# ztaylor797/APMBackend

Hardware: AMD Instinct MI355X
Metric: log-lines/sec z-scored (whole node) (higher is better)
Workload: dtype fp64

## Files before the change

apmbackend_amd/csrc/kernels/common.h:

```cpp
#pragma once
#include <cstring>
#include <cstdio>
#include <cstdlib>
#include <hip/hip_runtime.h>
#include <stdint.h>
#include <math.h>

#include "../apm_types.h"

#define APM_WAVE 64

#define HIP_OK(x)                                                                      \
  do {                                                                                 \
    hipError_t _e = (x);                                                               \
    if (_e != hipSuccess) {                                                            \
      fprintf(stderr, "HIP error %s at %s:%d: %s\n", hipGetErrorName(_e), __FILE__,    \
              __LINE__, hipGetErrorString(_e));                                        \
      abort();                                                                         \
    }                                                                                  \
  } while (0)

namespace apm {

__host__ __device__ inline double apm_nan() { return __builtin_nan(""); }
// ... 9 lines not shown
}

__host__ __device__ inline int64_t floordiv64(int64_t a, int64_t b) {
  int64_t q = a / b;
  if ((a % b != 0) && ((a < 0) != (b < 0))) --q;
  return q;
}

__host__ __device__ inline int64_t make_date_ms(int64_t y, int64_t mon0, int64_t d, int64_t h,
                                                int64_t mi, int64_t s, int64_t ms) {
  const int64_t ym = y + floordiv64(mon0, 12);
  const int64_t mn = mon0 - floordiv64(mon0, 12) * 12;
  const int64_t day = days_from_civil(ym, mn + 1, 1) + d - 1;
  return day * 86400000LL + ((h * 60 + mi) * 60 + s) * 1000 + ms;
}

struct TzTable {
  int n;
  int64_t local_start[64];
  int64_t offset_ms[64];
};

__host__ __device__ inline int64_t local_to_utc(const TzTable& tz, int64_t local_ms) {
  int lo = 0, hi = tz.n - 1;
  while (lo < hi) {
    int mid = (lo + hi + 1) >> 1;
    if (tz.local_start[mid] <= local_ms) lo = mid; else hi = mid - 1;
  }
  return local_ms - tz.offset_ms[lo];
}

__host__ __device__ inline double js_round_fixed(double x, int f) {
  if (x != x) return x;
  const double scale = f == 0 ? 1.0 : (f == 1 ? 10.0 : (f == 2 ? 100.0 : 1000.0));
  const bool neg = x < 0;
  const double ax = neg ? -x : x;
  if (ax >= 1e21) return x;
  const double p = ax * scale;
  const double e = fma(ax, scale, -p);
  const double q = floor(p);
  const double d = (p - q) - 0.5;
  double n = q;
  if (d > 0 || (d == 0 && e >= 0)) n = q + 1;
  double r = n / scale;
  return neg ? -r : r;
}

constexpr int HIST_BINS = 120;
__host__ __device__ inline int hist_bin(int32_t v) {
  if (v < 4) return v <= 0 ? 0 : v;
  const int e = 31 - __builtin_clz((uint32_t)v);
  return 4 * (e - 1) + (int)(((uint32_t)v >> (e - 2)) & 3u);
}
__host__ __device__ inline uint32_t hist_lower(int b) {
  return b < 4 ? (uint32_t)b : (uint32_t)(4 + (b & 3)) << (b / 4 - 1);
}

__host__ __device__ inline uint64_t hash_mix(uint64_t a, uint64_t b) {
  const __uint128_t r = (__uint128_t)a * b;
  return (uint64_t)r ^ (uint64_t)(r >> 64);
}

constexpr uint64_t kHashSeed = 0x243f6a8885a308d3ULL;
constexpr uint64_t kHashSeedEjb = 0x13198a2e03707344ULL;

__host__ __device__ inline uint64_t hash_bytes(const void* data, size_t n, uint64_t seed = kHashSeed) {
  const uint8_t* p = static_cast<const uint8_t*>(data);
  uint64_t h = seed ^ hash_mix(n ^ 0xa0761d6478bd642fULL, 0xe7037ed1a0b428dbULL);
  while (n >= 8) {
    uint64_t w;
    memcpy(&w, p, 8);
    h = hash_mix(h ^ w, 0x8ebc6af09c88c6e3ULL);
    p += 8;
    n -= 8;
  }
  if (n) {
    uint64_t w = 0;
    memcpy(&w, p, n);
    h = hash_mix(h ^ w ^ ((uint64_t)n << 59), 0x589965cc75374cc3ULL);
  }
  return hash_mix(h, 0x1d8e4e27c47d124fULL);
}

__host__ __device__ inline uint64_t fnv1a64(const uint8_t* p, int n, uint64_t h = 1469598103934665603ULL) {
  for (int i = 0; i < n; ++i) { h ^= p[i]; h *= 1099511628211ULL; }
  return h;
}

}
```

apmbackend_amd/csrc/kernels/devjoin.hip:

```cpp
#include "kernel_api.h"

#include <rocprim/rocprim.hpp>

#include <chrono>
#include <climits>
#include <cstdlib>
#include <cstddef>
#include <cstring>
#include <vector>

#include "devjoin_api.h"
#include "devjoin_dev.h"
#include "devscan.h"
#include "prim.h"
#include "textout.h"

namespace apm {
using namespace dj;

namespace {

constexpr int TB = 256;

__device__ __forceinline__ uint32_t grid_n(uint32_t n) { return (n + TB - 1) / TB; }

constexpr uint32_t AUD_NIL = 0xffffffffu;

__device__ __forceinline__ bool ws_ascii(uint8_t c) { return c == ' ' || (c >= 9 && c <= 13); }

__device__ __forceinline__ void trim_ascii(const uint8_t* p, int& a, int& b) {
  while (a < b && ws_ascii(p[a])) ++a;
  while (b > a && ws_ascii(p[b - 1])) --b;
}

__device__ bool parse_int_nobr(const uint8_t* p, int a, int b, double& out) {
  uint64_t x = 0;
  int nd = 0, k = 0;
  for (int i = a; i < b; ++i) {
    const uint8_t ch = p[i];
    if (ch == '[' || ch == ']') continue;
    if (k == 0 && (ch == '+' || ch == '-')) return false;
    if (k == 1 && nd == 1 && x == 0 && (ch == 'x' || ch == 'X')) return false;
    ++k;
    if (ch < '0' || ch > '9') break;
    if (nd >= 19) return false;
    x = x * 10 + (ch - '0');
    ++nd;
  }
  out = nd == 0 ? apm_nan() : (double)x;
  return true;
}

__device__ int aud_date(const uint8_t* p, int a, int b, double& out) {
  if (a >= b) return 1;
  int tpos = -1;
  for (int i = a; i < b; ++i) if (p[i] == 'T') { tpos = i; break; }
  bool iso = false;
  if (tpos >= 0) for (int i = tpos + 1; i < b; ++i) if (p[i] == '-') { iso = true; break; }
  if (!iso) return -1;
  trim_ascii(p, a, b);
  const int n = b - a;
  const uint8_t* t = p + a;
  auto dig = [&](int i, int k, int64_t& v) {
    if (i + k > n) return false;
    v = 0;
    for (int j = 0; j < k; ++j) {
      const uint8_t c = t[i + j];
      if (c < '0' || c > '9') return false;
      v = v * 10 + (c - '0');
    }
    return true;
  };
  out = apm_nan();
  int64_t y, mo, d, h, mi, sec = 0, ms = 0;
  if (!dig(0, 4, y) || n < 16 || t[4] != '-' || !dig(5, 2, mo) || t[7] != '-' || !dig(8, 2, d) || t[10] != 'T' ||
      !dig(11, 2, h) || t[13] != ':' || !dig(14, 2, mi))
    return 0;
  int i = 16;
  if (i < n && t[i] == ':') {
    if (!dig(i + 1, 2, sec)) return 0;
    i += 3;
    if (i < n && t[i] == '.') {
      ++i;
      int j = i, nd = 0;
      int64_t frac = 0;
      while (j < n && t[j] >= '0' && t[j] <= '9') { if (nd < 3) { frac = frac * 10 + (t[j] - '0'); ++nd; } ++j; }
      if (j == i) return 0;
      while (nd < 3) { frac *= 10; ++nd; }
      ms = frac;
      i = j;
    }
  }
  if (mo < 1 || mo > 12 || d < 1 || d > 31 || h > 24 || mi > 59 || sec > 59) return 0;
  const int64_t local = make_date_ms(y, mo - 1, d, h, mi, sec, ms);
  if (i == n) return -1;
  if (t[i] == 'Z' && i + 1 == n) { out = (double)local; return 0; }
  if (t[i] == '+' || t[i] == '-') {
    const int sg = t[i] == '-' ? -1 : 1;
    int64_t oh, om;
    if (!dig(i + 1, 2, oh)) return 0;
    int k = i + 3;
    if (k < n && t[k] == ':') ++k;
    if (!dig(k, 2, om) || k + 2 != n) return 0;
    out = (double)(local - sg * (oh * 60 + om) * 60000);
  }
  return 0;
}

__device__ bool icontains_provider(const uint8_t* p, int a, int b) {
  const char* pat = "provider[";
  for (int i = a; i + 9 <= b; ++i) {
    int k = 0;
    for (; k < 9; ++k) {
      uint8_t c = p[i + k];
      if (c >= 'A' && c <= 'Z') c = (uint8_t)(c + 32);
      if (c != (uint8_t)pat[k]) break;
    }
    if (k == 9) return true;
  }
  return false;
}

struct LineScan {
  bool nonascii;
  int c1, c2;
  int t0s, t0e, t3s, t3e, t5s, t5e;
  int eq1, eq2;
  int lt, gt;
};

__device__ void line_scan(const uint8_t* __restrict__ p, int len, LineScan& L) {
  bool na = false;
  int c1 = -1, c2 = len;
  int t0s = -1, t0e = -1, t3s = -1, t3e = -1, t5s = -1, t5e = -1;
  int eq1 = -1, eq2 = -1, lt = len, gt = -1;
  int tok = 0, tstart = 0;
  bool in_ws = false, lt_found = false;
  uint8_t prev = 0;
  const uintptr_t a0 = (uintptr_t)p & ~(uintptr_t)15;
  const int lead = (int)((uintptr_t)p - a0);
  for (int base = -lead; base < len; base += 16) {
    const uint4 v = *reinterpret_cast<const uint4*>(p + base);
    const uint32_t w4[4] = {v.x, v.y, v.z, v.w};
#pragma unroll
    for (int j = 0; j < 16; ++j) {
      const int i = base + j;
      if (i < 0 || i >= len) continue;
      const uint8_t c = (uint8_t)(w4[j >> 2] >> (8 * (j & 3)));
      na |= c >= 0x80;
      if (c == ':') {
        if (c1 < 0) c1 = i;
        else if (c2 == len) c2 = i;
      }
      if (!lt_found) {
        if (prev == '<' && c == '/') { lt = i - 1; lt_found = true; }
        else if (c == '>') gt = i;
      }
      if (ws_ascii(c)) {
        if (!in_ws) {
          if (tok == 0) { t0s = tstart; t0e = i; }
          else if (tok == 3) { t3s = tstart; t3e = i; }
          else if (tok == 5) { t5s = tstart; t5e = i; }
          ++tok;
          in_ws = true;
        }
        tstart = i + 1;
      } else {
        in_ws = false;
        if (tok == 5 && c == '=') {
          if (eq1 < 0) eq1 = i + 1;
          else if (eq2 < 0) eq2 = i;
        }
      }
      prev = c;
    }
  }
  if (tok == 0) { t0s = tstart; t0e = len; }
  else if (tok == 3) { t3s = tstart; t3e = len; }
  else if (tok == 5) { t5s = tstart; t5e = len; }
  if (eq1 >= 0 && eq2 < 0) eq2 = t5e;
  L.nonascii = na; L.c1 = c1; L.c2 = c2;
  L.t0s = t0s; L.t0e = t0e; L.t3s = t3s; L.t3e = t3e; L.t5s = t5s; L.t5e = t5e;
  L.eq1 = eq1; L.eq2 = eq2; L.lt = lt; L.gt = gt;
}

__device__ bool baf_account_scan(const uint8_t* p, int a, int b, int& n, bool& digits, double& v) {
  int st = a;
  for (int i = a; i + 1 < b; ++i) if (p[i] == ']' && p[i + 1] == '[') st = i + 2;
  int c = st;
  for (int i = st; i < b; ++i) if (p[i] == ':') c = i + 1;
  n = 0;
  digits = true;
  uint64_t x = 0;
  int nd = 0;
  bool in_digits = true;
  for (int i = c; i < b; ++i) {
    const uint8_t ch = p[i];
    if (ch == '[' || ch == ']') continue;
    const bool d = ch >= '0' && ch <= '9';
    if (n == 0 && (ch == '+' || ch == '-')) return false;
    if (n == 1 && nd == 1 && x == 0 && (ch == 'x' || ch == 'X')) return false;
    digits &= d;
    if (in_digits) {
      if (d) {
        if (nd >= 19) return false;
        x = x * 10 + (ch - '0');
        ++nd;
      } else {
        in_digits = false;
      }
    }
    ++n;
  }
  v = nd == 0 ? apm_nan() : (double)x;
  if (n == 0) digits = false;
  return true;
}

__device__ bool aud_fields(const Event& e, const uint8_t* __restrict__ p, uint64_t fkey, AudF& f) {
  const int len = (int)e.len;
  f.h_item = 0; f.el = apm_nan(); f.h_sw = 0; f.ts = apm_nan();
  f.ref = 0; f.len = 0; f.flags = 0; f.pad = 0; f.pad2[0] = f.pad2[1] = 0;
  LineScan L;
  line_scan(p, len, L);
  if (L.nonascii) return false;
  const uint32_t m = e.mask;
  if (m & PM_AUTR_MAP) {
    int s0 = L.t0s, e0 = L.t0e;
    if (s0 < 0) { s0 = e0 = 0; }
    if (s0 < e0 && p[s0] == '[') ++s0;
    if (e0 > s0 && p[e0 - 1] == ']') --e0;
    for (int i = s0; i < e0; ++i) if (p[i] == '[' || p[i] == ']') return false;
    f.ref = e.off + (uint32_t)s0;
    f.len = (uint16_t)(e0 - s0);
    f.h_sw = hash_bytes(p + s0, (size_t)(e0 - s0));
    const uint64_t ah = L.eq1 < 0 ? hash_bytes("undefined", 9) : hash_bytes(p + L.eq1, (size_t)(L.eq2 - L.eq1));
    f.h_item = aud_key(ah, fkey);
    if ((m & PM_BAF) && L.t3s >= 0 && L.t3e > L.t3s) {
      int n;
      bool digits;
      double v;
      if (!baf_account_scan(p, L.t3s, L.t3e, n, digits, v)) return false;
      if (n > 0) {
        f.el = v;
        f.flags |= AF_ACCT;
        if (digits) f.flags |= AF_ACCT_VALID;
      }
    }
    return true;
  }
  if (m & PM_AUTR_HDR) {
    if (L.c1 < 0) return false;
    int a = L.c1 + 1, b = L.c2;
    trim_ascii(p, a, b);
    f.h_item = aud_key(hash_bytes(p + a, (size_t)(b - a)), fkey);
    return true;
  }
  {
    int a = 0, b = L.c1 >= 0 ? L.c1 : len;
    trim_ascii(p, a, b);
    f.h_item = hash_bytes(p + a, (size_t)(b - a));
    if (L.c1 >= 0) {
      int t = L.c1 + 1;
      while (t < L.c2 && !ws_ascii(p[t])) ++t;
      if (!parse_int_nobr(p, L.c1 + 1, t, f.el)) return false;
    }
  }
  if (m & (PM_SW_NAME | PM_SW_STARTTS | PM_SW_STOPTS)) {
    const int t = L.lt, s = L.gt >= 0 ? L.gt + 1 : 0;
    if (m & PM_SW_NAME) {
      f.ref = e.off + (uint32_t)s;
      f.len = (uint16_t)(t - s);
      f.h_sw = hash_bytes(p + s, (size_t)(t - s));
      if (!icontains_provider(p, s, t)) f.flags |= AF_TO_DB;
    } else {
      const int r = aud_date(p, s, t, f.ts);
      if (r < 0) return false;
      if (r == 1) f.flags |= AF_TS_EMPTY;
    }
  }
  return true;
}

enum : uint8_t { PRE_BAF = 1, PRE_BAF_VALID = 2, PRE_SOAP_VALID = 4 };
__device__ __forceinline__ uint32_t zero_bytes(uint32_t x) {
  return ~((((x & 0x7f7f7f7fu) + 0x7f7f7f7fu) | x) | 0x7f7f7f7fu);
}
__device__ void angle_field2_dev(const uint8_t* __restrict__ p, int len, int& fs, int& fe) {
  auto ws = [](uint8_t c) { return c == ' ' || (c >= 9 && c <= 13); };
  int a = 0, b = len;
  while (a < b && ws(p[a])) ++a;
  while (b > a && ws(p[b - 1])) --b;
  fs = fe = -1;
  int seen = 0, start = -1;
  const int lead = (int)((uintptr_t)(p + a) & 15u);
  const uint4* q = reinterpret_cast<const uint4*>(p + a - lead);
  for (int g = a - lead; g < b; g += 16, ++q) {
    const uint4 v = *q;
    const uint32_t w[4] = {v.x, v.y, v.z, v.w};
#pragma unroll
    for (int k = 0; k < 4; ++k) {
      uint32_t m = zero_bytes(w[k] ^ 0x3c3c3c3cu) | zero_bytes(w[k] ^ 0x3e3e3e3eu);
      while (m) {
        const int i = g + 4 * k + (__builtin_ctz(m) >> 3);
        m &= m - 1;
        if (i < a || i >= b) continue;
        if (seen == 2) { fs = start; fe = i; return; }
        if (++seen == 2) start = i + 1;
      }
    }
  }
  if (seen == 2) { fs = start; fe = b; }
}

__device__ int pre_fields(const Event& e, const uint8_t* __restrict__ p, AudF& f) {
  if (e.mask & PM_HOST) return -1;
  f.h_item = 0; f.el = apm_nan(); f.h_sw = 0; f.ts = apm_nan(); f.ref = 0; f.len = 0; f.flags = 0; f.pad = 0;
  if (e.kind >= LK_EJB_ENTRY && e.kind <= LK_CT_EXIT) {
    if (!(e.mask & PM_KEYS) || e.ntok < 3) return -1;
    if (e.kind == LK_CT_EXIT && (e.mask & PM_BAF)) {
      int n = 9;
      bool digits = false;
      double v = apm_nan();
      if (e.ntok >= 4 && !baf_account_scan(p, e.t3s, e.t3e, n, digits, v)) return -1;
      f.el = v;
      f.flags = (uint8_t)((n > 0 ? PRE_BAF : 0) | (digits ? PRE_BAF_VALID : 0));
      return 1;
    }
    return 0;
  }
  if (e.kind == LK_SOAP) {
    const uint32_t m = e.mask;
    if (m & PM_SOAP_IN) {
      int s = -1, t = -1;
      if (e.ntok >= 2) {
        const int a0 = e.t1s, b0 = e.t1e;
        for (int k = a0; k < b0; ++k) if (p[k] == '=') { s = k + 1; break; }
        if (s >= 0) { t = b0; for (int k = s; k < b0; ++k) if (p[k] == '=') { t = k; break; } }
      }
      f.h_item = s >= 0 ? hash_bytes(p + s, (size_t)(t - s)) : hash_bytes("undefined", 9, kHashSeedEjb);
      return 1;
    }
    if (m & PM_SOAP_OUT) return 0;
    if (m & (PM_SOAP_ACCT | PM_SOAP_VALUE)) {
      if (!(m & PM_SOAP_ACCT) && (m & PM_SOAP_KEY)) return 0;
      int fs, fe;
      angle_field2_dev(p, (int)e.len, fs, fe);
      if (fs >= 0) {
        while (fs < fe && (p[fs] == ' ' || (p[fs] >= 9 && p[fs] <= 13))) ++fs;
        while (fe > fs && (p[fe - 1] == ' ' || (p[fe - 1] >= 9 && p[fe - 1] <= 13))) --fe;
        if (all_digits(p + fs, fe - fs)) {
          double v;
          if (!simple_parse_int(p + fs, fe - fs, v)) return -1;
          f.el = v;
          f.flags = PRE_SOAP_VALID;
        }
      }
      return 1;
    }
  }
  return 0;
}

enum : uint8_t { SEL_HOST = 1, SEL_MH = 2, SEL_WALK = 4 };

constexpr int SEL_MH_SHIFT = 22, SEL_WALK_SHIFT = 43;
__device__ __forceinline__ SelCount sel_unpack(uint64_t v) {
  return SelCount{(uint32_t)(v & ((1ull << SEL_MH_SHIFT) - 1)),
                  (uint32_t)((v >> SEL_MH_SHIFT) & ((1ull << (SEL_WALK_SHIFT - SEL_MH_SHIFT)) - 1)),
                  (uint32_t)(v >> SEL_WALK_SHIFT), 0u};
}

constexpr int HF_SLOT = 256;
constexpr int HF_PITCH = HF_SLOT + 16;

__device__ __forceinline__ bool hf_needs_bytes(const Event& e) {
  if (e.kind == LK_APP) return !(e.mask & PM_HOST);
  if (e.mask & PM_HOST) return false;
  if (e.kind == LK_CT_EXIT) return (e.mask & PM_KEYS) && e.ntok >= 3 && (e.mask & PM_BAF);
  if (e.kind == LK_SOAP) return (e.mask & (PM_SOAP_IN | PM_SOAP_ACCT | PM_SOAP_VALUE)) != 0;
  return false;
}

__device__ __forceinline__ uint8_t hf_fields(const Event& e, const uint8_t* __restrict__ p, uint64_t fkey, AudF* aud,
                                             uint32_t i) {
  uint8_t fl = 0;
  if (e.kind == LK_APP) {
    bool host = (e.mask & PM_HOST) != 0;
    if (!host) {
      AudF f;
      host = !aud_fields(e, p, fkey, f);
      if (!host) aud[i] = f;
    }
    if (host) fl |= SEL_HOST;
  } else {
    AudF f;
    const int r = pre_fields(e, p, f);
    if (r < 0) fl |= SEL_HOST;
    else if (r > 0) aud[i] = f;
  }
  return fl;
}

__device__ __forceinline__ uint32_t wave_append(bool want, uint32_t* counter) {
  const uint64_t m = __ballot(want);
  if (!m) return ~0u;
  const uint32_t lane = threadIdx.x & (APM_WAVE - 1);
  const uint32_t leader = (uint32_t)__ffsll((unsigned long long)m) - 1u;
  uint32_t base = 0;
  if (lane == leader) base = atomicAdd(counter, (uint32_t)__popcll(m));
  base = (uint32_t)__shfl((int)base, (int)leader, APM_WAVE);
  return want ? base + (uint32_t)__popcll(m & ((1ull << lane) - 1ull)) : ~0u;
}

__device__ __forceinline__ uint64_t sel_pack(uint8_t fl) {
  return (uint64_t)(fl & SEL_HOST) | ((fl & SEL_MH) ? 1ull << SEL_MH_SHIFT : 0ull) |
         ((fl & SEL_WALK) ? 1ull << SEL_WALK_SHIFT : 0ull);
}

__device__ __forceinline__ uint8_t app_bits(const Event& e) {
  if (e.kind != LK_APP) return 0;
  return (e.mask & PM_AUTR_MAP) ? SEL_MH : (uint8_t)(SEL_WALK | ((e.mask & PM_AUTR_HDR) ? SEL_MH : 0));
}

__device__ __forceinline__ uint8_t hf_event(const Event& e, uint32_t i, const uint8_t* __restrict__ bytes,
                                            const uint32_t* __restrict__ chunk_file,
                                            const uint64_t* __restrict__ file_fkey, AudF* __restrict__ aud,
                                            uint8_t* stage) {
  const uint64_t fkey = e.kind == LK_APP ? file_fkey[chunk_file[e.chunk]] : 0;
  const uint8_t* p = bytes + e.off;
  const uint32_t lead = e.off & 15u;
  const uint32_t nvec = (lead + e.len + 15u) >> 4;
  if (hf_needs_bytes(e) && nvec * 16u <= (uint32_t)HF_SLOT) {
    const uint4* __restrict__ src = reinterpret_cast<const uint4*>(bytes + (e.off - lead));
    uint4* dst = reinterpret_cast<uint4*>(stage + threadIdx.x * HF_PITCH);
    for (uint32_t k = 0; k < nvec; k += 4) {
      const uint4 v0 = src[k];
      const uint4 v1 = k + 1 < nvec ? src[k + 1] : v0;
      const uint4 v2 = k + 2 < nvec ? src[k + 2] : v0;
      const uint4 v3 = k + 3 < nvec ? src[k + 3] : v0;
      dst[k] = v0;
      if (k + 1 < nvec) dst[k + 1] = v1;
      if (k + 2 < nvec) dst[k + 2] = v2;
      if (k + 3 < nvec) dst[k + 3] = v3;
    }
    p = stage + threadIdx.x * HF_PITCH + lead;
  }
  return (uint8_t)(hf_fields(e, p, fkey, aud, i) | app_bits(e));
}

__global__ __launch_bounds__(TB) void k_host_flags(const Event* __restrict__ ev, const uint32_t* __restrict__ n_ev_dev,
                                                   const uint8_t* __restrict__ bytes,
                                                   uint8_t* __restrict__ flag, uint64_t* __restrict__ val,
                                                   AudF* __restrict__ aud, SelCount* __restrict__ totals, uint32_t cap,
                                                   uint32_t* __restrict__ list, uint32_t* __restrict__ list_n) {
  const uint32_t i = blockIdx.x * blockDim.x + threadIdx.x;
  const uint32_t n = min(*n_ev_dev, cap);
  if (blockIdx.x * blockDim.x >= n) return;
  uint32_t ab = 0;
  Event e;
  bool defer = false, front = false;
  if (i < n) {
    e = ev[i];
    if (e.kind == LK_APP && (e.mask & (PM_AUTR_MAP | PM_SW_NAME))) ab = e.len;
    defer = hf_needs_bytes(e);
    front = defer && e.kind == LK_APP;
  }
  const uint32_t f = wave_append(front, &list_n[0]);
  const uint32_t b = wave_append(defer && !front, &list_n[1]);
  if (front) list[f] = i;
  if (defer && !front) list[cap - 1 - b] = i;
  if (i < n && !defer) {
    const uint8_t fl = (uint8_t)(hf_fields(e, bytes + e.off, 0, aud, i) | app_bits(e));
    flag[i] = fl;
    val[i] = sel_pack(fl);
  }
  for (int o = APM_WAVE / 2; o > 0; o >>= 1) ab += __shfl_xor(ab, o, APM_WAVE);
  if ((threadIdx.x & (APM_WAVE - 1)) == 0 && ab) atomicAdd(&totals->aud_bytes, ab);
}

__global__ __launch_bounds__(TB) void k_host_flags_bytes(const Event* __restrict__ ev, const uint8_t* __restrict__ bytes,
                                                         const uint32_t* __restrict__ chunk_file,
                                                         const uint64_t* __restrict__ file_fkey,
                                                         uint8_t* __restrict__ flag, uint64_t* __restrict__ val,
                                                         AudF* __restrict__ aud, uint32_t cap,
                                                         const uint32_t* __restrict__ list,
                                                         const uint32_t* __restrict__ list_n) {
  __shared__ __attribute__((aligned(16))) uint8_t stage[TB * HF_PITCH];
  const uint32_t nf = list_n[0], nb = list_n[1];
  const uint32_t b0 = blockIdx.x * blockDim.x, b1 = b0 + blockDim.x;
  if (b0 >= nf && b1 <= cap - nb) return;
  const uint32_t t = b0 + threadIdx.x;
  if (t >= cap || (t >= nf && t < cap - nb)) return;
  const uint32_t i = list[t];
  const Event e = ev[i];
  const uint8_t fl = hf_event(e, i, bytes, chunk_file, file_fkey, aud, stage);
  flag[i] = fl;
  val[i] = sel_pack(fl);
}

struct SelValF {
  const uint64_t* val;
  __device__ uint64_t operator()(uint32_t i) const { return val[i]; }
};
struct SelScatterG {
  const Event* ev;
  const uint8_t* flag;
  const uint64_t* total;
  Event* out;
  uint32_t *out_idx, *mh_idx, *walk_idx;
  SelCount* totals;
  __device__ void operator()(uint32_t i, uint64_t pos) const {
    if (i == 0) {
      const SelCount t = sel_unpack(*total);
      totals->host = t.host; totals->mh = t.mh; totals->walk = t.walk;
    }
    const uint8_t fl = flag[i];
    if (!fl) return;
    const SelCount p = sel_unpack(pos);
    if (fl & SEL_HOST) { out[p.host] = ev[i]; out_idx[p.host] = i; }
    if (fl & SEL_MH) mh_idx[p.mh] = i;
    if (fl & SEL_WALK) walk_idx[p.walk] = i;
  }
};

enum : uint8_t { SC_NONE = 0, SC_IN = 1, SC_OUT = 2, SC_ACCT = 3, SC_KEY = 4, SC_VALUE = 5, SC_ACCT_BAD = 6,
                 SC_VALUE_BAD = 7 };

__device__ const HostOp* find_hop(const HostOp* __restrict__ h, uint32_t n, uint32_t ev) {
  uint32_t lo = 0, hi = n;
  while (lo < hi) {
    const uint32_t mid = (lo + hi) >> 1;
    if (h[mid].ev < ev) lo = mid + 1; else hi = mid;
  }
  return (lo < n && h[lo].ev == ev) ? &h[lo] : nullptr;
}

__global__ __launch_bounds__(TB) void k_build_ops(DJArgs a) {
  const uint32_t i = blockIdx.x * blockDim.x + threadIdx.x;
  if (i >= a.n_ev) return;
  const Event e = a.ev[i];
  JOp op;
  op.gkey = 0; op.svc = 0; op.ts = apm_nan(); op.num = apm_nan(); op.aux = apm_nan(); op.aux2 = apm_nan();
  op.line = e.line; op.lid = 0; op.svc_ref = 0; op.lid_len = 0; op.svc_len = 0;
  op.flags = 0; op.op = JOP_NONE; op.pad = 0;
  const int32_t file = (int32_t)a.chunk_file[e.chunk];
  const int32_t server = a.file_server[file];
  const uint64_t skey = a.file_skey[file];
  op.server = server;
  uint8_t code = SC_NONE;
  double snum = apm_nan();
  uint64_t shash = 0;
  const uint8_t* p = a.bytes + e.off;
  if (e.kind == LK_APP) {
    AudF f;
    bool ok = false;
    if (a.host_flag[i] & SEL_HOST) {
      const HostOp* h = find_hop(a.hops, a.n_hops, i);
      if (h && h->kind == HOP_AUD) { f = *reinterpret_cast<const AudF*>(&h->op); ok = true; }
      if (!ok) {
        f.h_item = 0; f.el = apm_nan(); f.h_sw = 0; f.ts = apm_nan(); f.ref = 0; f.len = 0; f.flags = 0;
      }
      a.aud[i] = f;
    } else {
      f = a.aud[i];
    }
    if ((e.mask & PM_AUTR_MAP) && (f.flags & AF_ACCT)) {
      if (!(f.flags & AF_ACCT_VALID)) {
        atomicAdd(&a.counts->invalid_acct, 1ULL);
      } else if (f.len > 0) {
        op.op = JOP_ACCT;
        op.gkey = gkey_of(f.h_sw, skey);
        op.num = f.el;
      }
    }
  } else if (a.host_flag[i] & SEL_HOST) {
    const HostOp* h = find_hop(a.hops, a.n_hops, i);
    if (h) {
      switch (h->kind) {
// ... 705 lines not shown
  ne.iblk = 0;
  ne.lblk = 0;
  ne.vidx = a.arena_base + k;
  uint32_t n = op.lid_len;
  const uint8_t* src = (op.flags & JF_LID_HOST) ? a.hbuf + op.lid
                      : (op.flags & JF_LID_AUD) ? (const uint8_t*)a.gin.txt + op.lid : a.bytes + op.lid;
  for (uint32_t j = 0; j < n && j < (uint32_t)NEED_LID; ++j) ne.lid[j] = (char)src[j];
  int32_t prev = 0;
  for (uint32_t o = NEED_LID; o < n; o += LBLK_N) {
    const int32_t b = blk_alloc(a);
    if (!b) { atomicAdd(&a.counts->need_overflow, 1ULL); n = o; break; }
    atomicAdd(&a.counts->chain_lids, 1ULL);
    if (prev) *(int32_t*)blk_ptr(a.pool, prev) = b;
    else ne.lblk = b;
    LidBlk* lb = (LidBlk*)blk_ptr(a.pool, b);
    const uint32_t m = min((uint32_t)LBLK_N, n - o);
    for (uint32_t j = 0; j < m; ++j) lb->b[j] = (char)src[o + j];
    prev = b;
  }
  ne.lid_len = (int32_t)n;
  return (int32_t)idx;
}

__device__ void need_put(DJArgs& a, NeedEnt& ne, const NeedItem& it) {
  const int n = ne.n;
  for (int j = 0; j < n && j < NEED_ITEMS; ++j)
    if (ne.items[j].svc == it.svc) { ne.items[j] = it; return; }
  if (n > NEED_ITEMS) {
    int j = NEED_ITEMS;
    for (int32_t b = ne.iblk; b && j < n; b = blk_next(a.pool, b)) {
      NeedBlk* nb = (NeedBlk*)blk_ptr(a.pool, b);
      for (int k = 0; k < NBLK_N && j < n; ++k, ++j)
        if (nb->items[k].svc == it.svc) { nb->items[k] = it; return; }
    }
  }
  if (n < NEED_ITEMS) { ne.items[n] = it; ne.n = n + 1; return; }
  const int j = n - NEED_ITEMS;
  int32_t b;
  if (j % NBLK_N == 0) {
    b = blk_alloc(a);
    if (!b) { atomicAdd(&a.counts->need_overflow, 1ULL); return; }
    atomicAdd(&a.counts->chain_items, 1ULL);
    if (j == 0) ne.iblk = b;
    else *(int32_t*)blk_ptr(a.pool, chain_at(a.pool, ne.iblk, j / NBLK_N - 1)) = b;
  } else {
    b = chain_at(a.pool, ne.iblk, j / NBLK_N);
  }
  ((NeedBlk*)blk_ptr(a.pool, b))->items[j % NBLK_N] = it;
  ne.n = n + 1;
}

__device__ __forceinline__ const NeedItem& need_item(const uint8_t* pool, const NeedEnt& ne, int j, int32_t& b) {
  if (j < NEED_ITEMS) return ne.items[j];
  const int k = (j - NEED_ITEMS) % NBLK_N;
  if (k == 0) b = (j == NEED_ITEMS) ? ne.iblk : blk_next(pool, b);
  return ((const NeedBlk*)blk_ptr(pool, b))->items[k];
}

__device__ void need_drain(DJArgs& a, NeedEnt& ne, int32_t nidx, double acct, Emitter& em) {
  int32_t b = 0;
  for (int j = 0; j < ne.n; ++j) {
    const NeedItem& r = need_item(a.pool, ne, j, b);
    em.put(make_tx(ne.server, r.svc, LID_NEED, (uint32_t)nidx, (uint32_t)ne.lid_len, acct, r.start,
                   (r.flags & JF_START_EMPTY) != 0, r.end, (r.flags & JF_TS_EMPTY) != 0, r.elapsed, false));
  }
  if (ne.iblk) chain_free(a.pool, a.pool_ring, a.pool_mask, a.counts, ne.iblk);
  ne.iblk = 0;
  ne.n = 0;
}

__device__ __forceinline__ void walk_direct(const DJArgs& a, uint32_t ev) {
  const JOp op = a.ops[ev];
  Emitter em{a.stage, a.ovf, &a.counts->pad[0], ev, 0};
  em.put(make_tx(op.server, op.svc, LID_NONE, 0, 0, (op.flags & JF_BAF) ? op.aux : apm_nan(), 0.0, true, op.ts,
                 (op.flags & JF_TS_EMPTY) != 0, op.num, false));
  a.out_cnt[ev] = em.sub;
}

template <class M>
__device__ void walk_group(DJArgs& a, uint32_t slot, const M& mem, uint32_t g);

constexpr uint32_t GW_SMALL = 16;
struct GwRow {
  uint32_t m[GW_SMALL];
  __device__ __forceinline__ void clear() {
#pragma unroll
    for (uint32_t k = 0; k < GW_SMALL; ++k) m[k] = ~0u;
  }
  __device__ __forceinline__ void insert(uint32_t j) {
#pragma unroll
    for (uint32_t k = GW_SMALL - 1; k >= 1; --k) m[k] = min(m[k], max(m[k - 1], j));
    m[0] = min(m[0], j);
  }
  __device__ __forceinline__ uint32_t at(uint32_t q) const {
    uint32_t v = m[0];
#pragma unroll
    for (uint32_t k = 1; k < GW_SMALL; ++k) v = q == k ? m[k] : v;
    return v;
  }
};
__global__ __launch_bounds__(TB) void k_group_walk(DJArgs a) {
  const uint32_t i = blockIdx.x * blockDim.x + threadIdx.x;
  if (i >= a.n_ev) return;
  const uint32_t cap = a.table_mask + 1;
  const uint32_t slot = a.op_slot[i];
  if (slot > cap) return;
  if (slot == cap) { walk_direct(a, i); return; }
  if (a.op_idx[i] != ~0u) return;
  GwRow m;
  m.clear();
  uint32_t g = 0;
  for (uint32_t j = a.slot_head[slot]; j != ~0u; j = a.op_idx[j]) {
    if (g == GW_SMALL) {
      a.op_slot_sorted[atomicAdd(&a.big[0], 1u)] = slot;
      return;
    }
    ++g;
    m.insert(j);
  }
  a.slot_head[slot] = ~0u;
  walk_group(a, slot, [&m](uint32_t q) { return m.at(q); }, g);
}

__device__ void block_sort_asc(uint32_t* v, uint32_t g) {
  uint32_t np2 = 1;
  while (np2 < g) np2 <<= 1;
  for (uint32_t k = 2; k <= np2; k <<= 1) {
    for (uint32_t j = k >> 1; j > 0; j >>= 1) {
      for (uint32_t t = threadIdx.x; t < np2 / 2; t += blockDim.x) {
        uint32_t lo, hi;
        if (j == (k >> 1)) {
          lo = (t / j) * k + t % j;
          hi = (t / j) * k + k - 1 - t % j;
        } else {
          lo = (t / j) * 2 * j + t % j;
          hi = lo + j;
        }
        if (hi < g) {
          const uint32_t x = v[lo], y = v[hi];
          if (x > y) { v[lo] = y; v[hi] = x; }
        }
      }
      __syncthreads();
    }
  }
}

constexpr uint32_t GWB_LDS = 4096;
constexpr int GWB_THREADS = 256;
__global__ __launch_bounds__(GWB_THREADS) void k_group_walk_big(DJArgs a) {
  __shared__ uint32_t lds[GWB_LDS];
  __shared__ uint32_t s_g, s_off;
  const uint32_t nb = a.big[0];
  for (uint32_t b = blockIdx.x; b < nb; b += gridDim.x) {
    const uint32_t slot = a.op_slot_sorted[b];
    if (threadIdx.x == 0) {
      uint32_t g = 0;
      for (uint32_t j = a.slot_head[slot]; j != ~0u; j = a.op_idx[j]) ++g;
      const uint32_t off = atomicAdd(&a.big[1], g);
      uint32_t k = 0;
      for (uint32_t j = a.slot_head[slot]; j != ~0u; j = a.op_idx[j]) a.op_idx_sorted[off + k++] = j;
      a.slot_head[slot] = ~0u;
      s_g = g;
      s_off = off;
    }
    __syncthreads();
    const uint32_t g = s_g;
    uint32_t* v = a.op_idx_sorted + s_off;
    if (g <= GWB_LDS) {
      for (uint32_t t = threadIdx.x; t < g; t += blockDim.x) lds[t] = v[t];
      __syncthreads();
      v = lds;
    }
    block_sort_asc(v, g);
    if (threadIdx.x == 0) walk_group(a, slot, [v](uint32_t q) { return v[q]; }, g);
    __syncthreads();
  }
}

template <class M>
__device__ void walk_group(DJArgs& a, uint32_t slot, const M& mem, uint32_t g) {
  KeyState ks = a.table[slot];
  const double now = a.now;
  bool acct_live = ks.acct_exp >= now;
  if (!(ks.rec_exp >= now) && ks.n_part > 0) {
    atomicAdd(&a.counts->expired_partials, (unsigned long long)ks.n_part);
    part_clear(a, ks);
  }
  NeedEnt* ne = nullptr;
  int32_t nidx = -1;
  if (ks.need >= 0) {
    NeedEnt* c = &a.arena[ks.need];
    if (c->key == ks.key && c->exp >= now) { ne = c; nidx = ks.need; }
  }
  for (uint32_t q = 0; q < g; ++q) {
    const uint32_t ev = mem(q);
    const JOp op = a.ops[ev];
    Emitter em{a.stage, a.ovf, &a.counts->pad[0], ev, 0};
    const bool ts_empty = (op.flags & JF_TS_EMPTY) != 0;
    switch (op.op) {
      case JOP_ENTRY: {
        if (!(ks.rec_exp >= now)) { ks.rec_exp = now + a.rec_ttl; part_clear(a, ks); }
        const int f = part_find(a, ks, op.svc);
        if (f >= 0) part_set(a, ks, f, op.svc, op.ts);
// ... 1189 lines not shown
```

apmbackend_amd/csrc/kernels/devjoin_dev.h:

```cpp
#pragma once
#include "common.h"
#include "devjoin_types.h"

namespace apm {
namespace dj {

__host__ __device__ inline uint64_t gkey_of(uint64_t lid_hash, uint64_t skey) {
  const uint64_t k = hash_mix(lid_hash ^ (skey * 0x9E3779B97F4A7C15ULL), 0xd6e8feb86659fd93ULL);
  return k ? k : 1;
}
__host__ __device__ inline uint64_t server_key_of(const char* name, size_t n) {
  return hash_bytes(name, n, 0x5e7e7e7e5e7e7e7eULL) | 1ULL;
}
__host__ __device__ inline uint64_t file_key_of(const char* path, size_t n) {
  return hash_bytes(path, n, 0xf11ef11ef11ef11eULL) | 1ULL;
}
__host__ __device__ inline uint64_t regkey_of(uint64_t svc, int32_t server) {
  const uint64_t k = hash_mix(svc ^ ((uint64_t)(uint32_t)(server + 7) * 0xC2B2AE3D27D4EB4FULL), 0x165667b19e3779f9ULL);
  return k ? k : 1;
}
__host__ __device__ inline uint64_t aud_key(uint64_t autr_hash, uint64_t fkey) {
  return hash_mix(autr_hash, 0x9e3779b97f4a7c15ULL + fkey) | 1ULL;
}
__host__ __device__ inline uint32_t home_of(uint64_t k, uint32_t mask) {
// ... 29 lines not shown
    const int nd = u64_digits(v);
    if (p) {
      if (neg) p[0] = '-';
      u64_write(p + (neg ? 1 : 0), v, nd);
    }
    return nd + (neg ? 1 : 0);
  }
  char buf[64];
  char* o = p ? p : buf;
  int n = 0;
  if (neg) { o[n++] = '-'; x = ax; }
  if (x == __builtin_inf()) {
    const char* s = "Infinity";
    for (int i = 0; i < 8; ++i) o[n + i] = s[i];
    return n + 8;
  }
  if (x < 1.7014118346046923e38 && x == floor(x)) {
    int e2;
    const double fr = frexp(x, &e2);
    (void)fr;
    const unsigned __int128 M = (unsigned __int128)x;
    const int sh = e2 - 53;
    const unsigned __int128 ulp = (unsigned __int128)1 << sh;
    const bool pow2 = (M & (M - 1)) == 0;
    const unsigned __int128 hi = ulp >> 1;
    const unsigned __int128 lo = pow2 ? (ulp >> 2) : (ulp >> 1);
    const bool even = ((M >> sh) & 1) == 0;
    auto inside = [&](unsigned __int128 c) {
      if (c >= M) { const unsigned __int128 d = c - M; return d < hi || (d == hi && even); }
      const unsigned __int128 d = M - c;
      return d < lo || (d == lo && even);
    };
    unsigned __int128 best = M, p10 = 1;
    for (int k = 1; k < 39; ++k) {
      const unsigned __int128 q = p10 * 10;
      if (q > M) break;
      const unsigned __int128 down = M - M % q, up = down + q;
      const bool di = inside(down), ui = inside(up);
      if (!di && !ui) break;
      unsigned __int128 c;
      if (di && ui) {
        const unsigned __int128 dd = M - down, du = up - M;
        c = dd < du ? down : (du < dd ? up : (((down / q) & 1) == 0 ? down : up));
      } else {
        c = di ? down : up;
      }
      best = c;
      p10 = q;
    }
    char d[48];
    int nd = put_dec(d, best);
    int tz = 0;
    while (nd - tz > 1 && d[nd - 1 - tz] == '0') ++tz;
    const int exp10 = nd - 1;
    if (exp10 < 21) {
      for (int i = 0; i < nd; ++i) o[n + i] = d[i];
      return n + nd;
    }
    const int k = nd - tz;
    o[n++] = d[0];
    if (k > 1) { o[n++] = '.'; for (int i = 1; i < k; ++i) o[n++] = d[i]; }
    o[n++] = 'e'; o[n++] = '+';
    n += put_dec(o + n, (unsigned __int128)exp10);
    return n;
  }
  if (inexact) *inexact = true;
  int e10 = 0;
  double y = x;
  while (y >= 10.0) { y /= 10.0; ++e10; }
  while (y < 1.0) { y *= 10.0; --e10; }
  uint64_t m = (uint64_t)(y * 1e16 + 0.5);
  if (m >= 100000000000000000ULL) { m /= 10; ++e10; }
  char d[24];
  int nd = put_dec(d, m);
  while (nd > 1 && d[nd - 1] == '0') --nd;
  o[n++] = d[0];
  if (nd > 1) { o[n++] = '.'; for (int i = 1; i < nd; ++i) o[n++] = d[i]; }
  o[n++] = 'e';
  o[n++] = e10 >= 0 ? '+' : '-';
  n += put_dec(o + n, (unsigned __int128)(e10 >= 0 ? e10 : -e10));
  return n;
}

__host__ __device__ inline bool simple_parse_int(const uint8_t* s, int n, double& out) {
  if (n > 0 && (s[0] == '+' || s[0] == '-')) return false;
  if (n >= 2 && s[0] == '0' && (s[1] == 'x' || s[1] == 'X')) return false;
  uint64_t v = 0;
  int nd = 0;
  while (nd < n && s[nd] >= '0' && s[nd] <= '9') {
    if (nd >= 19) return false;
    v = v * 10 + (uint64_t)(s[nd] - '0');
    ++nd;
  }
  out = nd == 0 ? __builtin_nan("") : (double)v;
  return true;
}

__host__ __device__ inline bool all_digits(const uint8_t* s, int n) {
  if (n <= 0) return false;
  for (int i = 0; i < n; ++i)
    if (s[i] < '0' || s[i] > '9') return false;
  return true;
}

__host__ __device__ inline int baf_account(const uint8_t* p, int a, int b, uint8_t* out) {
  int s = a;
  for (int i = a; i + 1 < b; ++i)
    if (p[i] == ']' && p[i + 1] == '[') s = i + 2;
  int c = s;
  for (int i = s; i < b; ++i)
    if (p[i] == ':') c = i + 1;
  int n = 0;
  for (int i = c; i < b; ++i) {
    if (p[i] == '[' || p[i] == ']') continue;
    if (n >= 64) return -1;
    out[n++] = p[i];
  }
  return n;
}

}
}
```

Baseline: 313.6 million.

## Stage line bytes in column-major LDS and move group-walk row to LDS

Replaces the per-thread row-major shared staging buffer for line bytes with a column-major word layout (stride TB), so lanes accessing the same word index hit different banks. All parsing helpers are templated over a line view (flat global pointer or LDS-staged view) with custom hashing and unaligned loads from the staged words. Separately, the group-walk per-thread 16-entry sorted array moves from registers to a column-major LDS array with insertion sort, cutting register pressure at the cost of LDS traffic. The byte-extraction arithmetic for the staged view adds ALU work per access.

```diff
diff --git a/apmbackend_amd/csrc/kernels/common.h b/apmbackend_amd/csrc/kernels/common.h
--- a/apmbackend_amd/csrc/kernels/common.h
+++ b/apmbackend_amd/csrc/kernels/common.h
@@ -115,6 +115,19 @@
   return hash_mix(h, 0x1d8e4e27c47d124fULL);
 }
 
+template <class Load>
+__host__ __device__ inline uint64_t hash_bytes_via(const Load& load, size_t n, uint64_t seed = kHashSeed) {
+  uint64_t h = seed ^ hash_mix(n ^ 0xa0761d6478bd642fULL, 0xe7037ed1a0b428dbULL);
+  size_t off = 0;
+  while (n >= 8) {
+    h = hash_mix(h ^ load(off, 8), 0x8ebc6af09c88c6e3ULL);
+    off += 8;
+    n -= 8;
+  }
+  if (n) h = hash_mix(h ^ load(off, (int)n) ^ ((uint64_t)n << 59), 0x589965cc75374cc3ULL);
+  return hash_mix(h, 0x1d8e4e27c47d124fULL);
+}
+
 __host__ __device__ inline uint64_t fnv1a64(const uint8_t* p, int n, uint64_t h = 1469598103934665603ULL) {
   for (int i = 0; i < n; ++i) { h ^= p[i]; h *= 1099511628211ULL; }
   return h;
diff --git a/apmbackend_amd/csrc/kernels/devjoin.hip b/apmbackend_amd/csrc/kernels/devjoin.hip
--- a/apmbackend_amd/csrc/kernels/devjoin.hip
+++ b/apmbackend_amd/csrc/kernels/devjoin.hip
@@ -24,16 +24,72 @@
 
 __device__ __forceinline__ uint32_t grid_n(uint32_t n) { return (n + TB - 1) / TB; }
 
+struct FlatLine {
+  const uint8_t* __restrict__ p;
+  __device__ __forceinline__ uint8_t operator[](int i) const { return p[i]; }
+  __device__ __forceinline__ int misalign(int i) const { return (int)((uintptr_t)(p + i) & 15u); }
+  __device__ __forceinline__ uint4 vec16(int i) const { return *reinterpret_cast<const uint4*>(p + i); }
+  struct Blocks {
+    const uint4* q;
+    __device__ __forceinline__ uint4 operator*() const { return *q; }
+    __device__ __forceinline__ void operator++() { ++q; }
+  };
+  __device__ __forceinline__ Blocks blocks(int i) const { return Blocks{reinterpret_cast<const uint4*>(p + i)}; }
+  __device__ __forceinline__ FlatLine at(int i) const { return FlatLine{p + i}; }
+  __device__ __forceinline__ uint64_t hash(int i, size_t n, uint64_t seed = kHashSeed) const {
+    return hash_bytes(p + i, n, seed);
+  }
+};
+
+typedef const __attribute__((address_space(3))) uint32_t lds_cu32;
+struct StageLine {
+  lds_cu32* col;
+  uint32_t o;
+  __device__ __forceinline__ uint32_t word(uint32_t k) const { return col[k * TB]; }
+  __device__ __forceinline__ uint8_t operator[](int i) const {
+    const uint32_t a = o + (uint32_t)i;
+    return (uint8_t)(word(a >> 2) >> (8 * (a & 3u)));
+  }
+  __device__ __forceinline__ int misalign(int i) const { return (int)((o + (uint32_t)i) & 15u); }
+  __device__ __forceinline__ uint4 vec16(int i) const {
+    const uint32_t k = (o + (uint32_t)i) >> 2;
+    return make_uint4(word(k), word(k + 1), word(k + 2), word(k + 3));
+  }
+  struct Blocks {
+    lds_cu32* r;
+    __device__ __forceinline__ uint4 operator*() const { return make_uint4(r[0], r[TB], r[2 * TB], r[3 * TB]); }
+    __device__ __forceinline__ void operator++() { r += 4 * TB; }
+  };
+  __device__ __forceinline__ Blocks blocks(int i) const { return Blocks{col + ((o + (uint32_t)i) >> 2) * TB}; }
+  __device__ __forceinline__ StageLine at(int i) const { return StageLine{col, o + (uint32_t)i}; }
+  __device__ __forceinline__ uint64_t load_le(size_t off, int k) const {
+    const uint32_t a = o + (uint32_t)off, d = a >> 2, dl = (a + (uint32_t)k - 1u) >> 2, sh = 8 * (a & 3u);
+    const uint32_t w0 = word(d);
+    const uint32_t w1 = d + 1 <= dl ? word(d + 1) : 0u;
+    const uint32_t w2 = d + 2 <= dl ? word(d + 2) : 0u;
+    const uint64_t lo = ((uint64_t)w1 << 32) | w0;
+    uint64_t v = lo >> sh;
+    if (sh) v |= (uint64_t)w2 << (64 - sh);
+    return k == 8 ? v : v & ((1ull << (8 * k)) - 1ull);
+  }
+  __device__ __forceinline__ uint64_t hash(int i, size_t n, uint64_t seed = kHashSeed) const {
+    const StageLine s = at(i);
+    return hash_bytes_via([s](size_t off, int k) { return s.load_le(off, k); }, n, seed);
+  }
+};
+
 constexpr uint32_t AUD_NIL = 0xffffffffu;
 
 __device__ __forceinline__ bool ws_ascii(uint8_t c) { return c == ' ' || (c >= 9 && c <= 13); }
 
-__device__ __forceinline__ void trim_ascii(const uint8_t* p, int& a, int& b) {
+template <class V>
+__device__ __forceinline__ void trim_ascii(const V p, int& a, int& b) {
   while (a < b && ws_ascii(p[a])) ++a;
   while (b > a && ws_ascii(p[b - 1])) --b;
 }
 
-__device__ bool parse_int_nobr(const uint8_t* p, int a, int b, double& out) {
+template <class V>
+__device__ bool parse_int_nobr(const V p, int a, int b, double& out) {
   uint64_t x = 0;
   int nd = 0, k = 0;
   for (int i = a; i < b; ++i) {
@@ -51,7 +107,8 @@
   return true;
 }
 
-__device__ int aud_date(const uint8_t* p, int a, int b, double& out) {
+template <class V>
+__device__ int aud_date(const V p, int a, int b, double& out) {
   if (a >= b) return 1;
   int tpos = -1;
   for (int i = a; i < b; ++i) if (p[i] == 'T') { tpos = i; break; }
@@ -60,7 +117,7 @@
   if (!iso) return -1;
   trim_ascii(p, a, b);
   const int n = b - a;
-  const uint8_t* t = p + a;
+  const V t = p.at(a);
   auto dig = [&](int i, int k, int64_t& v) {
     if (i + k > n) return false;
     v = 0;
@@ -107,7 +164,8 @@
   return 0;
 }
 
-__device__ bool icontains_provider(const uint8_t* p, int a, int b) {
+template <class V>
+__device__ bool icontains_provider(const V p, int a, int b) {
   const char* pat = "provider[";
   for (int i = a; i + 9 <= b; ++i) {
     int k = 0;
@@ -129,7 +187,8 @@
   int lt, gt;
 };
 
-__device__ void line_scan(const uint8_t* __restrict__ p, int len, LineScan& L) {
+template <class V>
+__device__ void line_scan(const V p, int len, LineScan& L) {
   bool na = false;
   int c1 = -1, c2 = len;
   int t0s = -1, t0e = -1, t3s = -1, t3e = -1, t5s = -1, t5e = -1;
@@ -137,10 +196,9 @@
   int tok = 0, tstart = 0;
   bool in_ws = false, lt_found = false;
   uint8_t prev = 0;
-  const uintptr_t a0 = (uintptr_t)p & ~(uintptr_t)15;
-  const int lead = (int)((uintptr_t)p - a0);
+  const int lead = p.misalign(0);
   for (int base = -lead; base < len; base += 16) {
-    const uint4 v = *reinterpret_cast<const uint4*>(p + base);
+    const uint4 v = p.vec16(base);
     const uint32_t w4[4] = {v.x, v.y, v.z, v.w};
 #pragma unroll
     for (int j = 0; j < 16; ++j) {
@@ -184,7 +242,8 @@
   L.eq1 = eq1; L.eq2 = eq2; L.lt = lt; L.gt = gt;
 }
 
-__device__ bool baf_account_scan(const uint8_t* p, int a, int b, int& n, bool& digits, double& v) {
+template <class V>
+__device__ bool baf_account_scan(const V p, int a, int b, int& n, bool& digits, double& v) {
   int st = a;
   for (int i = a; i + 1 < b; ++i) if (p[i] == ']' && p[i + 1] == '[') st = i + 2;
   int c = st;
@@ -217,7 +276,8 @@
   return true;
 }
 
-__device__ bool aud_fields(const Event& e, const uint8_t* __restrict__ p, uint64_t fkey, AudF& f) {
+template <class V>
+__device__ bool aud_fields(const Event& e, const V p, uint64_t fkey, AudF& f) {
   const int len = (int)e.len;
   f.h_item = 0; f.el = apm_nan(); f.h_sw = 0; f.ts = apm_nan();
   f.ref = 0; f.len = 0; f.flags = 0; f.pad = 0; f.pad2[0] = f.pad2[1] = 0;
@@ -233,8 +293,8 @@
     for (int i = s0; i < e0; ++i) if (p[i] == '[' || p[i] == ']') return false;
     f.ref = e.off + (uint32_t)s0;
     f.len = (uint16_t)(e0 - s0);
-    f.h_sw = hash_bytes(p + s0, (size_t)(e0 - s0));
-    const uint64_t ah = L.eq1 < 0 ? hash_bytes("undefined", 9) : hash_bytes(p + L.eq1, (size_t)(L.eq2 - L.eq1));
+    f.h_sw = p.hash(s0, (size_t)(e0 - s0));
+    const uint64_t ah = L.eq1 < 0 ? hash_bytes("undefined", 9) : p.hash(L.eq1, (size_t)(L.eq2 - L.eq1));
     f.h_item = aud_key(ah, fkey);
     if ((m & PM_BAF) && L.t3s >= 0 && L.t3e > L.t3s) {
       int n;
@@ -253,13 +313,13 @@
     if (L.c1 < 0) return false;
     int a = L.c1 + 1, b = L.c2;
     trim_ascii(p, a, b);
-    f.h_item = aud_key(hash_bytes(p + a, (size_t)(b - a)), fkey);
+    f.h_item = aud_key(p.hash(a, (size_t)(b - a)), fkey);
     return true;
   }
   {
     int a = 0, b = L.c1 >= 0 ? L.c1 : len;
     trim_ascii(p, a, b);
-    f.h_item = hash_bytes(p + a, (size_t)(b - a));
+    f.h_item = p.hash(a, (size_t)(b - a));
     if (L.c1 >= 0) {
       int t = L.c1 + 1;
       while (t < L.c2 && !ws_ascii(p[t])) ++t;
@@ -271,7 +331,7 @@
     if (m & PM_SW_NAME) {
       f.ref = e.off + (uint32_t)s;
       f.len = (uint16_t)(t - s);
-      f.h_sw = hash_bytes(p + s, (size_t)(t - s));
+      f.h_sw = p.hash(s, (size_t)(t - s));
       if (!icontains_provider(p, s, t)) f.flags |= AF_TO_DB;
     } else {
       const int r = aud_date(p, s, t, f.ts);
@@ -286,15 +346,16 @@
 __device__ __forceinline__ uint32_t zero_bytes(uint32_t x) {
   return ~((((x & 0x7f7f7f7fu) + 0x7f7f7f7fu) | x) | 0x7f7f7f7fu);
 }
-__device__ void angle_field2_dev(const uint8_t* __restrict__ p, int len, int& fs, int& fe) {
+template <class V>
+__device__ void angle_field2_dev(const V p, int len, int& fs, int& fe) {
   auto ws = [](uint8_t c) { return c == ' ' || (c >= 9 && c <= 13); };
   int a = 0, b = len;
   while (a < b && ws(p[a])) ++a;
   while (b > a && ws(p[b - 1])) --b;
   fs = fe = -1;
   int seen = 0, start = -1;
-  const int lead = (int)((uintptr_t)(p + a) & 15u);
-  const uint4* q = reinterpret_cast<const uint4*>(p + a - lead);
+  const int lead = p.misalign(a);
+  auto q = p.blocks(a - lead);
   for (int g = a - lead; g < b; g += 16, ++q) {
     const uint4 v = *q;
     const uint32_t w[4] = {v.x, v.y, v.z, v.w};
@@ -313,7 +374,8 @@
   if (seen == 2) { fs = start; fe = b; }
 }
 
-__device__ int pre_fields(const Event& e, const uint8_t* __restrict__ p, AudF& f) {
+template <class V>
+__device__ int pre_fields(const Event& e, const V p, AudF& f) {
   if (e.mask & PM_HOST) return -1;
   f.h_item = 0; f.el = apm_nan(); f.h_sw = 0; f.ts = apm_nan(); f.ref = 0; f.len = 0; f.flags = 0; f.pad = 0;
   if (e.kind >= LK_EJB_ENTRY && e.kind <= LK_CT_EXIT) {
@@ -338,7 +400,7 @@
         for (int k = a0; k < b0; ++k) if (p[k] == '=') { s = k + 1; break; }
         if (s >= 0) { t = b0; for (int k = s; k < b0; ++k) if (p[k] == '=') { t = k; break; } }
       }
-      f.h_item = s >= 0 ? hash_bytes(p + s, (size_t)(t - s)) : hash_bytes("undefined", 9, kHashSeedEjb);
+      f.h_item = s >= 0 ? p.hash(s, (size_t)(t - s)) : hash_bytes("undefined", 9, kHashSeedEjb);
       return 1;
     }
     if (m & PM_SOAP_OUT) return 0;
@@ -349,9 +411,9 @@
       if (fs >= 0) {
         while (fs < fe && (p[fs] == ' ' || (p[fs] >= 9 && p[fs] <= 13))) ++fs;
         while (fe > fs && (p[fe - 1] == ' ' || (p[fe - 1] >= 9 && p[fe - 1] <= 13))) --fe;
-        if (all_digits(p + fs, fe - fs)) {
+        if (all_digits(p.at(fs), fe - fs)) {
           double v;
-          if (!simple_parse_int(p + fs, fe - fs, v)) return -1;
+          if (!simple_parse_int(p.at(fs), fe - fs, v)) return -1;
           f.el = v;
           f.flags = PRE_SOAP_VALID;
         }
@@ -372,7 +434,6 @@
 }
 
 constexpr int HF_SLOT = 256;
-constexpr int HF_PITCH = HF_SLOT + 16;
 
 __device__ __forceinline__ bool hf_needs_bytes(const Event& e) {
   if (e.kind == LK_APP) return !(e.mask & PM_HOST);
@@ -382,8 +443,8 @@
   return false;
 }
 
-__device__ __forceinline__ uint8_t hf_fields(const Event& e, const uint8_t* __restrict__ p, uint64_t fkey, AudF* aud,
-                                             uint32_t i) {
+template <class V>
+__device__ __forceinline__ uint8_t hf_fields(const Event& e, const V p, uint64_t fkey, AudF* aud, uint32_t i) {
   uint8_t fl = 0;
   if (e.kind == LK_APP) {
     bool host = (e.mask & PM_HOST) != 0;
@@ -426,27 +487,31 @@
 __device__ __forceinline__ uint8_t hf_event(const Event& e, uint32_t i, const uint8_t* __restrict__ bytes,
                                             const uint32_t* __restrict__ chunk_file,
                                             const uint64_t* __restrict__ file_fkey, AudF* __restrict__ aud,
-                                            uint8_t* stage) {
+                                            __attribute__((address_space(3))) uint32_t* col) {
   const uint64_t fkey = e.kind == LK_APP ? file_fkey[chunk_file[e.chunk]] : 0;
-  const uint8_t* p = bytes + e.off;
   const uint32_t lead = e.off & 15u;
   const uint32_t nvec = (lead + e.len + 15u) >> 4;
   if (hf_needs_bytes(e) && nvec * 16u <= (uint32_t)HF_SLOT) {
     const uint4* __restrict__ src = reinterpret_cast<const uint4*>(bytes + (e.off - lead));
-    uint4* dst = reinterpret_cast<uint4*>(stage + threadIdx.x * HF_PITCH);
+    auto put = [col](uint32_t k, const uint4& v) {
+      col[(4 * k + 0) * TB] = v.x;
+      col[(4 * k + 1) * TB] = v.y;
+      col[(4 * k + 2) * TB] = v.z;
+      col[(4 * k + 3) * TB] = v.w;
+    };
     for (uint32_t k = 0; k < nvec; k += 4) {
       const uint4 v0 = src[k];
       const uint4 v1 = k + 1 < nvec ? src[k + 1] : v0;
       const uint4 v2 = k + 2 < nvec ? src[k + 2] : v0;
       const uint4 v3 = k + 3 < nvec ? src[k + 3] : v0;
-      dst[k] = v0;
-      if (k + 1 < nvec) dst[k + 1] = v1;
-      if (k + 2 < nvec) dst[k + 2] = v2;
-      if (k + 3 < nvec) dst[k + 3] = v3;
-    }
-    p = stage + threadIdx.x * HF_PITCH + lead;
-  }
-  return (uint8_t)(hf_fields(e, p, fkey, aud, i) | app_bits(e));
+      put(k, v0);
+      if (k + 1 < nvec) put(k + 1, v1);
+      if (k + 2 < nvec) put(k + 2, v2);
+      if (k + 3 < nvec) put(k + 3, v3);
+    }
+    return (uint8_t)(hf_fields(e, StageLine{col, lead}, fkey, aud, i) | app_bits(e));
+  }
+  return (uint8_t)(hf_fields(e, FlatLine{bytes + e.off}, fkey, aud, i) | app_bits(e));
 }
 
 __global__ __launch_bounds__(TB) void k_host_flags(const Event* __restrict__ ev, const uint32_t* __restrict__ n_ev_dev,
@@ -471,7 +536,7 @@
   if (front) list[f] = i;
   if (defer && !front) list[cap - 1 - b] = i;
   if (i < n && !defer) {
-    const uint8_t fl = (uint8_t)(hf_fields(e, bytes + e.off, 0, aud, i) | app_bits(e));
+    const uint8_t fl = (uint8_t)(hf_fields(e, FlatLine{bytes + e.off}, 0, aud, i) | app_bits(e));
     flag[i] = fl;
     val[i] = sel_pack(fl);
   }
@@ -486,7 +551,7 @@
                                                          AudF* __restrict__ aud, uint32_t cap,
                                                          const uint32_t* __restrict__ list,
                                                          const uint32_t* __restrict__ list_n) {
-  __shared__ __attribute__((aligned(16))) uint8_t stage[TB * HF_PITCH];
+  __shared__ uint32_t stage[HF_SLOT / 4][TB];
   const uint32_t nf = list_n[0], nb = list_n[1];
   const uint32_t b0 = blockIdx.x * blockDim.x, b1 = b0 + blockDim.x;
   if (b0 >= nf && b1 <= cap - nb) return;
@@ -494,7 +559,8 @@
   if (t >= cap || (t >= nf && t < cap - nb)) return;
   const uint32_t i = list[t];
   const Event e = ev[i];
-  const uint8_t fl = hf_event(e, i, bytes, chunk_file, file_fkey, aud, stage);
+  const uint8_t fl = hf_event(e, i, bytes, chunk_file, file_fkey, aud,
+                              (__attribute__((address_space(3))) uint32_t*)&stage[0][threadIdx.x]);
   flag[i] = fl;
   val[i] = sel_pack(fl);
 }
@@ -1366,24 +1432,21 @@
 
 constexpr uint32_t GW_SMALL = 16;
 struct GwRow {
-  uint32_t m[GW_SMALL];
-  __device__ __forceinline__ void clear() {
-#pragma unroll
-    for (uint32_t k = 0; k < GW_SMALL; ++k) m[k] = ~0u;
-  }
-  __device__ __forceinline__ void insert(uint32_t j) {
-#pragma unroll
-    for (uint32_t k = GW_SMALL - 1; k >= 1; --k) m[k] = min(m[k], max(m[k - 1], j));
-    m[0] = min(m[0], j);
-  }
-  __device__ __forceinline__ uint32_t at(uint32_t q) const {
-    uint32_t v = m[0];
-#pragma unroll
-    for (uint32_t k = 1; k < GW_SMALL; ++k) v = q == k ? m[k] : v;
-    return v;
+  __attribute__((address_space(3))) uint32_t* col;
+  __device__ __forceinline__ uint32_t at(uint32_t q) const { return col[q * TB]; }
+  __device__ __forceinline__ void insert(uint32_t g, uint32_t j) {
+    uint32_t k = g;
+#pragma unroll 1
+    for (; k > 0; --k) {
+      const uint32_t v = col[(k - 1) * TB];
+      if (v < j) break;
+      col[k * TB] = v;
+    }
+    col[k * TB] = j;
   }
 };
 __global__ __launch_bounds__(TB) void k_group_walk(DJArgs a) {
+  __shared__ uint32_t row[GW_SMALL][TB];
   const uint32_t i = blockIdx.x * blockDim.x + threadIdx.x;
   if (i >= a.n_ev) return;
   const uint32_t cap = a.table_mask + 1;
@@ -1391,19 +1454,19 @@
   if (slot > cap) return;
   if (slot == cap) { walk_direct(a, i); return; }
   if (a.op_idx[i] != ~0u) return;
-  GwRow m;
-  m.clear();
+  GwRow m{(__attribute__((address_space(3))) uint32_t*)&row[0][threadIdx.x]};
   uint32_t g = 0;
+#pragma unroll 1
   for (uint32_t j = a.slot_head[slot]; j != ~0u; j = a.op_idx[j]) {
     if (g == GW_SMALL) {
       a.op_slot_sorted[atomicAdd(&a.big[0], 1u)] = slot;
       return;
     }
+    m.insert(g, j);
     ++g;
-    m.insert(j);
   }
   a.slot_head[slot] = ~0u;
-  walk_group(a, slot, [&m](uint32_t q) { return m.at(q); }, g);
+  walk_group(a, slot, [m](uint32_t q) { return m.at(q); }, g);
 }
 
 __device__ void block_sort_asc(uint32_t* v, uint32_t g) {
diff --git a/apmbackend_amd/csrc/kernels/devjoin_dev.h b/apmbackend_amd/csrc/kernels/devjoin_dev.h
--- a/apmbackend_amd/csrc/kernels/devjoin_dev.h
+++ b/apmbackend_amd/csrc/kernels/devjoin_dev.h
@@ -135,7 +135,8 @@
   return n;
 }
 
-__host__ __device__ inline bool simple_parse_int(const uint8_t* s, int n, double& out) {
+template <class S>
+__host__ __device__ inline bool simple_parse_int(const S& s, int n, double& out) {
   if (n > 0 && (s[0] == '+' || s[0] == '-')) return false;
   if (n >= 2 && s[0] == '0' && (s[1] == 'x' || s[1] == 'X')) return false;
   uint64_t v = 0;
@@ -149,7 +150,8 @@
   return true;
 }
 
-__host__ __device__ inline bool all_digits(const uint8_t* s, int n) {
+template <class S>
+__host__ __device__ inline bool all_digits(const S& s, int n) {
   if (n <= 0) return false;
   for (int i = 0; i < n; ++i)
     if (s[i] < '0' || s[i] > '9') return false;
```

After: 296.8 million. 5.4% lower.
